# AvalonEnjoyer/pytorch-ViT-paper-replication

Hardware: AMD Instinct MI355X
Metric: images/sec (whole node) ViT-B/16 224px bf16 at 1/2/4/8 MI355X (higher is better)
Workload: dtype bf16; 1 GPU; model=ViT-B/16, global_batch=256, per_gpu_batch=256, seq_len=197, image_size=224, parallelism=dp1, impl=fused, grad_transport=none, optimizer=Adam(wd=0.03 decay group) + clip 1.0 + warmup/linear-decay LR, dropout=0.1 (mlp, embedding)

## Files before the change

### pytorch_vit_paper_replication_amd/csrc/bindings.cpp

```cpp
#include <cstdlib>
#include <algorithm>
#include <map>
#include <torch/extension.h>
#include <c10/hip/HIPStream.h>
#include <hip/hip_runtime.h>

#include "kernels.h"

namespace {

hipStream_t stream() { return c10::hip::getCurrentHIPStream().stream(); }
using ScratchKey = std::pair<int, int64_t>;
ScratchKey scratch_key(int dev) { return std::make_pair(dev, (int64_t)c10::hip::getCurrentHIPStream().id()); }
template <class T>
std::map<ScratchKey, T>& scratch_map() {
  static auto* m = new std::map<ScratchKey, T>();
  return *m;
}
struct SkCounters { torch::Tensor t; };
struct DetWs { torch::Tensor t; };
struct DqWs { torch::Tensor t; };
struct AttnWs { torch::Tensor t; };

int num_cus() {
// ... 931 lines not shown
  TORCH_CHECK(D % H == 0 && pvr_attn_cls_ok((int)N, (int)(D / H)), "attn_cls_fwd: unsupported N / head dim (attn_cls_ok)");
  auto out = torch::empty({B, D}, qkv.options());
  auto lse = torch::empty({B * H}, qkv.options().dtype(torch::kFloat32));
  check(pvr_attn_cls_fwd(bf(qkv, "qkv"), ld_of(qkv, "qkv"), bf_mut(out, "out"), D, f32_mut(lse, "lse"), (int)B, (int)N, (int)H, (int)D,
                         (float)scale, stream()),
        "attn_cls_fwd");
  return {out, lse};
}

std::vector<torch::Tensor> attn_cls_bwd(torch::Tensor dout, torch::Tensor qkv, torch::Tensor out, torch::Tensor lse, int64_t B, int64_t N,
                                        int64_t H, double scale) {
  TORCH_CHECK(qkv.dim() == 2 && qkv.size(0) == B * N && qkv.size(1) % 3 == 0 && H > 0, "attn_cls_bwd: qkv [B*N][3D]");
  const int64_t D = qkv.size(1) / 3;
  TORCH_CHECK(D % H == 0 && pvr_attn_cls_ok((int)N, (int)(D / H)), "attn_cls_bwd: unsupported N / head dim (attn_cls_ok)");
  TORCH_CHECK(dout.dim() == 2 && dout.size(0) == B && dout.size(1) == D && out.dim() == 2 && out.size(0) == B && out.size(1) == D &&
                  lse.numel() == B * H && lse.is_contiguous(),
              "attn_cls_bwd: dout / out [B][D], lse [B*H]");
  auto dqkv = torch::empty({B * N, 3 * D}, qkv.options());
  auto dq0 = torch::empty({B, D}, qkv.options().dtype(torch::kFloat32));
  check(pvr_attn_cls_bwd(bf(qkv, "qkv"), ld_of(qkv, "qkv"), bf(out, "out"), ld_of(out, "out"), bf(dout, "dout"), ld_of(dout, "dout"),
                         f32(lse, "lse"), bf_mut(dqkv, "dqkv"), 3 * D, f32_mut(dq0, "dq0"), (int)B, (int)N, (int)H, (int)D, (float)scale,
                         stream()),
        "attn_cls_bwd");
  return {dqkv, dq0};
}

void attn_cls_dbias(torch::Tensor dq0, torch::Tensor dout, torch::Tensor dbias) {
  TORCH_CHECK(dq0.dim() == 2 && dq0.is_contiguous() && dout.dim() == 2 && dout.size(0) == dq0.size(0) && dout.size(1) == dq0.size(1) &&
                  dbias.is_contiguous() && dbias.numel() == 3 * dq0.size(1),
              "attn_cls_dbias: dq0 f32 [B][D] contiguous, dout bf16 [B][D], dbias f32 [3D]");
  check(pvr_attn_cls_dbias(f32(dq0, "dq0"), bf(dout, "dout"), ld_of(dout, "dout"), f32_mut(dbias, "dbias"), (int)dq0.size(0),
                           (int)dq0.size(1), stream()),
        "attn_cls_dbias");
}

}

extern "C" const char* pvr_src_hash(void);

PYBIND11_MODULE(TORCH_EXTENSION_NAME, m) {
  m.doc() = "MI355X (gfx950) HIP kernels for pytorch_vit_paper_replication_amd";
  m.def("source_hash", []() { return std::string(pvr_src_hash()); },
        "content hash of the csrc/ sources this binary was built from (build.source_hash())");
  m.def("gemm_tail_split", [](int64_t M, int64_t N, int64_t K, int64_t elem_bytes, int64_t max_units) {
    return pvr_gemm_tail_split((int)M, (int)N, (int)K, (int)elem_bytes, (int)max_units); },
    py::arg("M"), py::arg("N"), py::arg("K"), py::arg("elem_bytes"), py::arg("max_units") = 0,
    "K-parts of the split tail round this GEMM shape gets (0: none)");
  m.def("set_attn_dbg", [](torch::Tensor t) { pvr_set_attn_dbg(t.defined() && t.numel() ? t.data_ptr() : nullptr); },
        "diagnostic builds (-DPVR_ATTN_STAMPS): int64 buffer for the attention backward's phase stamps "
        "[workgroup * waves + wave][8] (scripts/attn_stamps.py); a no-op otherwise");
  m.def("set_attn_prep_xcd", &pvr_set_attn_prep_xcd, "attention backward pre-pass: XCD-contiguous (batch, head) pairs (1) or round-robin (0, default); A/B");
  m.def("set_ln_fwd_q8_grid", &pvr_set_ln_fwd_q8_grid, "LayerNorm forward with the e4m3 copy: grid cap in workgroups per CU (A/B)");
  m.def("set_attn_fwd_head_qf", &pvr_set_attn_fwd_head_qf, "whole-head attention forward (dh 64, N <= 256): 16-query fragments per wave (1 = default, 2 = half the LDS reads with 7 waves; A/B)");
  m.def("set_attn_fwd_qg", &pvr_set_attn_fwd_qg, "tiled attention forward: 16-query groups per wave (0 = auto by query padding, 1 = round-3 form, 2 = forced; A/B)");
  m.def("set_fp8_persistent", &pvr_set_fp8_persistent, "fp8 fwd/dgrad GEMMs on the persistent ping-pong: 1 when the epilogue has no per-row input (default), 0 never (A/B)");
  m.def("set_deterministic", &set_deterministic, "deterministic reductions (partial rows + ordered sum) instead of float atomics");
  m.def("deterministic", &deterministic);
  m.def("set_gemm_tail", &set_gemm_tail, "split-K tail of the last dispatch round on (True, default) / off (A/B)");
  m.def("gemm", &gemm,py::arg("A"), py::arg("a_kcontig"), py::arg("B"), py::arg("b_kcontig"), py::arg("C"),
        py::arg("M"), py::arg("N"), py::arg("K"), py::arg("epi"), py::arg("bias"), py::arg("resid"), py::arg("addend"),
        py::arg("addend_period"), py::arg("aux"), py::arg("row_group"), py::arg("row_stride_group"),
        py::arg("row_offset"), py::arg("seed"), py::arg("seed_offset"), py::arg("drop_p"), py::arg("k_split"),
        py::arg("tile_cfg"), py::arg("dbg") = py::none(), py::arg("colsum") = py::none(),
        py::arg("epi_staged") = 0, py::arg("tail_limit") = 0, py::arg("reduce_out") = py::none(), py::arg("reduce_acc") = true,
        py::arg("drop_row_mul") = 0);
  m.def("splitk_timeouts", &splitk_timeouts, py::arg("like"), py::arg("reset") = false);
// ... 40 lines not shown
  m.def("metrics_accum", &metrics_accum);
  m.def("rng_next", &rng_next);
  m.def("zero_f32", &zero_f32);
  m.def("gemm_fp8", &gemm_fp8, py::arg("A"), py::arg("fmt_a"), py::arg("B"), py::arg("fmt_b"), py::arg("C"), py::arg("M"),
        py::arg("N"), py::arg("K"), py::arg("epi"), py::arg("scale_a"), py::arg("scale_b"), py::arg("bias") = py::none(),
        py::arg("resid") = py::none(), py::arg("aux") = py::none(), py::arg("seed") = py::none(), py::arg("seed_offset") = 0,
        py::arg("drop_p") = 0.0, py::arg("colsum") = py::none(), py::arg("q_out") = py::none(), py::arg("q_scale") = py::none(),
        py::arg("q_amax") = py::none(), py::arg("q_fmt") = 0, py::arg("c_skip") = false, py::arg("tail_limit") = 0);
  m.def("fp8_transpose", &fp8_transpose);
  m.def("gemm_fp8_wgrad_mn", &gemm_fp8_wgrad_mn, py::arg("dy8"), py::arg("x8"), py::arg("ws"), py::arg("N"), py::arg("K"),
        py::arg("T"), py::arg("scale_a"), py::arg("scale_b"), py::arg("ksplit"), py::arg("fmt_a") = 1);
  m.def("fp8_quant", &fp8_quant, py::arg("x"), py::arg("y"), py::arg("qscale"), py::arg("amax"), py::arg("fmt"));
  m.def("fp8_dequant", &fp8_dequant, py::arg("x"), py::arg("dscale") = py::none(), py::arg("fmt") = 0);
  m.def("fp8_scale_update", &fp8_scale_update);
  m.def("fp8_quant_t", &fp8_quant_t);
  m.def("gemm_fp8_wgrad", &gemm_fp8_wgrad, py::arg("A8"), py::arg("B8"), py::arg("ws"), py::arg("N"), py::arg("K"), py::arg("Tp"),
        py::arg("scale_a"), py::arg("scale_b"), py::arg("ksplit"), py::arg("fmt_a") = 1);
  m.def("fp8_quant_multi", &fp8_quant_multi, py::arg("segs"), py::arg("nchunks"), py::arg("qscale"), py::arg("amax"), py::arg("fmt"),
        py::arg("amax_only"));
  m.def("attn_fwd", &attn_fwd, py::arg("qkv"), py::arg("B"), py::arg("N"), py::arg("H"), py::arg("scale"),
        py::arg("seed") = py::none(), py::arg("seed_offset") = 0, py::arg("drop_p") = 0.0, py::arg("q_out") = py::none(),
        py::arg("q_scale") = py::none(), py::arg("q_amax") = py::none(), py::arg("q_only") = false);
  m.def("attn_bwd", &attn_bwd, py::arg("dout"), py::arg("qkv"), py::arg("out"), py::arg("lse"), py::arg("B"), py::arg("N"),
        py::arg("H"), py::arg("scale"), py::arg("dbias") = py::none(), py::arg("dbias_part") = py::none(),
        py::arg("seed") = py::none(), py::arg("seed_offset") = 0, py::arg("drop_p") = 0.0, py::arg("q_out") = py::none(),
        py::arg("q_scale") = py::none(), py::arg("q_amax") = py::none(), py::arg("q_only") = false,
        py::arg("q_fmt") = 1);
  m.def("attn_cls_ok", [](int64_t N, int64_t dh) { return pvr_attn_cls_ok((int)N, (int)dh) != 0; },
        "the class-token attention kernels take this token count and head dim");
  m.def("attn_cls_fwd", &attn_cls_fwd, py::arg("qkv"), py::arg("B"), py::arg("N"), py::arg("H"), py::arg("scale"));
  m.def("attn_cls_bwd", &attn_cls_bwd, py::arg("dout"), py::arg("qkv"), py::arg("out"), py::arg("lse"), py::arg("B"), py::arg("N"),
        py::arg("H"), py::arg("scale"));
  m.def("attn_cls_dbias", &attn_cls_dbias);
  m.def("attn_bwd_q8_ok", &attn_bwd_q8_ok, "attn_bwd can write dQKV's e5m2 copy for this shape");
  m.def("arch", []() { return std::string("gfx950"); });
}
```

### pytorch_vit_paper_replication_amd/csrc/kernels.h

```cpp
#pragma once
#include <stdint.h>

#include <hip/hip_runtime_api.h>

#include "gemm_params.h"

namespace pvr {

struct AdamGroup {
  float lr, beta1, beta2, eps, weight_decay;
  float bc1, bc2_sqrt;
  int decoupled;
};
static_assert(sizeof(AdamGroup) == 8 * sizeof(float), "AdamGroup is one float32 [8] row of the group table");

struct DropSite {
  const uint64_t* seed = nullptr; uint64_t offset = 0; uint32_t thr = 0; float scale = 1.f;
};

struct Fp8Copy {
  uint8_t* out = nullptr; int64_t ld = 0; const float* scale = nullptr; unsigned* amax = nullptr; int fmt = 0;
};

struct MixRow {
// ... 107 lines not shown
                               int amax_only, hipStream_t s);
hipError_t pvr_fp8_quant_t(const uint16_t* x, int64_t ldx, uint8_t* y, int64_t ldy, int T, int C, const float* qscale, int fmt,
                           hipStream_t s);
hipError_t pvr_fp8_transpose(const uint8_t* x, int64_t ldx, uint8_t* y, int64_t ldy, int T, int C, hipStream_t s);
hipError_t pvr_fp8_dequant(const uint8_t* x, float* y, int64_t n, const float* dscale, int fmt, hipStream_t s);
hipError_t pvr_fp8_scale_update(float* hist, int H, unsigned* amax, float* qscale, float* dscale, const float* fmax, int s0, int s1,
                                float margin_mul, hipStream_t s);

void pvr_set_attn_fwd_qg(int qg);
void pvr_set_attn_fwd_head_qf(int qf);
void pvr_set_attn_prep_xcd(int on);
void pvr_set_attn_dbg(void* p);
int pvr_attn_head_dim_supported(int dh);
hipError_t pvr_attn_fwd(const uint16_t* qkv, int64_t ld, uint16_t* out, int64_t ld_o, float* lse, int B, int N, int H, int D,
                        float scale, pvr::DropSite drop, pvr::Fp8Copy q8, int q8_only, hipStream_t s);
int pvr_attn_dbias_splits(int B, int NQ);
hipError_t pvr_attn_dbias_reduce(const float* part, float* ws, float* dbias, int B, int H, int NQ, int D, hipStream_t s);
int pvr_attn_bwd_waves(int N);
int pvr_attn_bwd_key_blocks(int N);
int pvr_attn_bwd_needs_dq_acc(int N, int dh, int dbias, int drop, int det);
int64_t pvr_attn_bwd_ws_floats(int B, int N, int H, int D, int dbias, int drop, int det);
int pvr_attn_bwd_q8_ok(int N, int drop);
int pvr_attn_bwd_uses_pipe(int B, int N, int H, int D, int64_t ld, int64_t ld_do, int64_t ld_o, int64_t ld_dq, int drop);
int pvr_attn_bwd_part_rows(int B, int N, int H, int D, int64_t ld, int64_t ld_do, int64_t ld_o, int64_t ld_dq, int drop);
hipError_t pvr_attn_bwd(const pvr::AttnBwdParams* p, hipStream_t s);
int pvr_attn_cls_ok(int N, int dh);
hipError_t pvr_attn_cls_fwd(const uint16_t* qkv, int64_t ld, uint16_t* out, int64_t ld_o, float* lse, int B, int N, int H, int D,
                            float scale, hipStream_t s);
hipError_t pvr_attn_cls_bwd(const uint16_t* qkv, int64_t ld, const uint16_t* o, int64_t ld_o, const uint16_t* dout, int64_t ld_do,
                            const float* lse, uint16_t* dqkv, int64_t ld_dq, float* dq0, int B, int N, int H, int D, float scale,
                            hipStream_t s);
hipError_t pvr_attn_cls_dbias(const float* dq0, const uint16_t* dout, int64_t ld_do, float* dbias, int B, int D, hipStream_t s);

}
```

### pytorch_vit_paper_replication_amd/ops/fused_vit.py

```python
from __future__ import annotations

import math
from typing import List, Optional

import torch
import torch.nn.functional as F

from .. import _ext
from . import gemm

SITE_SHIFT = 32
ATTN_SITE = 1 << 20


DGRAD_TAP = None


def site_drop(seed: Optional[torch.Tensor], site: int, p: float, training: bool):
    if seed is None or not training or p <= 0.0:
        return None
    return (seed, site << SITE_SHIFT, float(p))


def _patch_geometry(C, H, W, patch):
# ... 346 lines not shown
        if q8res is not None:
            pre_q[3] = q8res
        elif fp8_qkv:
            prod = f8d[0].grad_producer(f8d[1], 3)
            if side_db and prod is not None:
                pre_q[3] = gemm.bias_grad(dqkv, gbqkv, quant=prod)
                side_db = False
            else:
                pre_q[3] = f8d[0].grad_quant(dqkv, f8d[1], 3)
        store.on_side(attn_wgrads, dx1, o, dqkv, xn1, do, *(() if db_part is None else (db_part,)), *side8(2, 3))
        dxn1 = dgrad(dqkv, wqkv, 3)
        dx = torch.empty_like(dx2)
        if prev is not None:
            seed, soff, p = gemm._drop_args(prev.drop2)
            dzp = torch.empty_like(dx2) if seed is not None else None
            pf8 = (f8d[0], f8d[1] - 1) if f8d is not None and f8d[1] > 0 else None
            q_kw, q_dz = _ln_grad_quant(pf8, 0, dx.shape, dx.device)
            dz_nostore = (q_dz is not None and dzp is not None and T >= 256 and DGRAD_TAP is None
                          and prev.w2 is not None and store.bf16_t(prev.w2) is not None
                          and pf8[0].wgrad_ready(pf8[1], 0, 3))
            ext.layernorm_bwd(dxn1, D, x, D, mean1, rstd1, ln1w, dx1, D, dx, D, g(ln1w), g(ln1b), T,
                              dsum=g(prev.b2), dz=dzp, seed=seed, seed_offset=soff, drop_p=p, dz_nostore=dz_nostore, **q_kw)
            if dzp is not None:
                _poison(dzp, dz_nostore)
            prev.dz2, prev.dz2_q, prev.done = dzp, q_dz, True
        else:
            ext.layernorm_bwd(dxn1, D, x, D, mean1, rstd1, ln1w, dx1, D, dx, D, g(ln1w), g(ln1b), T)
        store.grad_ready([bo, wo, bqkv, wqkv, ln1w, ln1b])
        return (dx,) + (None,) * (9 + len(params))


CLS_LAST_BLOCK = True


def cls_last_block_ok(N: int, H: int, D: int, f8, dropa) -> bool:
    return (CLS_LAST_BLOCK and f8 is None and gemm._drop_args(dropa)[0] is None
            and D % H == 0 and bool(_ext.ext().attn_cls_ok(N, D // H)))


class EncoderBlockClsFn(torch.autograd.Function):

    @staticmethod
    def forward(ctx, x, B, N, H, eps1, eps2, store, drops, links, *params):
        ext = _ext.ext()
        drop1, drop2, _ = drops
        ln1w, ln1b, wqkv, bqkv, wo, bo, ln2w, ln2b, w1, b1, w2, b2 = params
        T, D = x.shape
        ctx.links = links if links is not None else (None, None)
        M = w1.shape[0]
        scale = 1.0 / math.sqrt(D // H)
        need_bwd = getattr(store, "grad_enabled", True) and any(ctx.needs_input_grad)
        xn1, mean1, rstd1 = ext.layernorm_fwd(x, ln1w, ln1b, eps1, T, D)
        qkv = gemm.linear_fwd(xn1, store.bf16(wqkv), bqkv)
        o, lse = ext.attn_cls_fwd(qkv, B, N, H, scale)
        xc = x.view(B, N, D)[:, 0]
        x1 = gemm.linear_fwd(o, store.bf16(wo), bo, resid=xc)
        xn2, mean2, rstd2 = ext.layernorm_fwd(x1, ln2w, ln2b, eps2, B, D)
        u = torch.empty(B, M, dtype=torch.bfloat16, device=x.device) if need_bwd else None
        h = gemm.linear_fwd(xn2, store.bf16(w1), b1, gelu_aux=u, gelu=True, drop=drop1, drop_row_mul=N)
        x2 = gemm.linear_fwd(h, store.bf16(w2), b2, resid=x1, drop=drop2, drop_row_mul=N)
        if need_bwd:
            ctx.save_for_backward(x, xn1, mean1, rstd1, qkv, o, lse, x1, xn2, mean2, rstd2, u, h)
        ctx.meta = (B, N, H, scale, store, drop2, params)
        return x2

    @staticmethod
    def backward(ctx, dx2):
        ext = _ext.ext()
        det = _ext.deterministic()
        x, xn1, mean1, rstd1, qkv, o, lse, x1, xn2, mean2, rstd2, u, h = ctx.saved_tensors
        B, N, H, scale, store, drop2, params = ctx.meta
        ln1w, ln1b, wqkv, bqkv, wo, bo, ln2w, ln2b, w1, b1, w2, b2 = params
        g = store.grad_dest
        dx2 = dx2.contiguous()
        T, D = x.shape
        _, prev = ctx.links

        def dgrad(dy, w, which, dgelu_aux=None, colsum=None):
            out = gemm.linear_dgrad(dy, store.bf16(w), dgelu_aux=dgelu_aux, wt=store.bf16_t(w), colsum=colsum)
            if DGRAD_TAP is not None:
                DGRAD_TAP(which, out)
            return out

        if drop2 is not None:
            dz2 = torch.empty_like(dx2)
            gemm.bias_grad(dx2, g(b2), drop=drop2, dz=dz2, row_mul=N)
        else:
            dz2 = dx2
            if b2.requires_grad:
                gemm.bias_grad(dx2, g(b2))
        gb1 = g(b1)
        gw2, gw1 = g(w2), g(w1)
        du = dgrad(dz2, w2, 0, dgelu_aux=u, colsum=None if det else gb1)
        if det and gb1 is not None:
            gemm.bias_grad(du, gb1)

        def mlp_wgrads():
            if gw2 is not None:
                gemm.linear_wgrad(dz2, h, gw2)
            if gw1 is not None:
                gemm.linear_wgrad(du, xn2, gw1)

        store.on_side(mlp_wgrads, dz2, h, du, xn2)
        dxn2 = dgrad(du, w1, 1)
        dx1 = torch.empty_like(dx2)
        ext.layernorm_bwd(dxn2, D, x1, D, mean2, rstd2, ln2w, dx2, D, dx1, D, g(ln2w), g(ln2b), B, dsum=g(bo))
        store.grad_ready([w2, b2, w1, b1, ln2w, ln2b])
        gwo, gwqkv, gbqkv = g(wo), g(wqkv), g(bqkv)
        do = dgrad(dx1, wo, 2)
        dqkv, dq0 = ext.attn_cls_bwd(do, qkv, o, lse, B, N, H, scale)

        def attn_wgrads():
            if gbqkv is not None:
                ext.attn_cls_dbias(dq0, do, gbqkv.view(-1))
            if gwo is not None:
                gemm.linear_wgrad(dx1, o, gwo)
            if gwqkv is not None:
                gemm.linear_wgrad(dqkv, xn1, gwqkv)

        store.on_side(attn_wgrads, dx1, o, dqkv, xn1, do, dq0)
        dxn1 = dgrad(dqkv, wqkv, 3)
        dx = torch.empty_like(x)
        if prev is not None:
            seed, soff, p = gemm._drop_args(prev.drop2)
            dzp = torch.empty_like(x) if seed is not None else None
            ext.layernorm_bwd(dxn1, D, x, D, mean1, rstd1, ln1w, dx1, D, dx, D, g(ln1w), g(ln1b), T,
                              dsum=g(prev.b2), dz=dzp, seed=seed, seed_offset=soff, drop_p=p, dres_every=N)
            prev.dz2, prev.dz2_q, prev.done = dzp, None, True
        else:
            ext.layernorm_bwd(dxn1, D, x, D, mean1, rstd1, ln1w, dx1, D, dx, D, g(ln1w), g(ln1b), T, dres_every=N)
        store.grad_ready([bo, wo, bqkv, wqkv, ln1w, ln1b])
        return (dx,) + (None,) * (8 + len(params))


class HeadFn(torch.autograd.Function):

    @staticmethod
    def forward(ctx, tokens, B, N, eps, store, ln_w, ln_b, head_w, head_b):
        ext = _ext.ext()
        logits, xhat, rstd = ext.head_fwd(tokens, B, N, ln_w, ln_b, eps, head_w, head_b)
        ctx.save_for_backward(xhat, rstd)
        ctx.meta = (B, N, store, ln_w, ln_b, head_w, head_b)
        return logits

    @staticmethod
    def backward(ctx, dlogits):
        ext = _ext.ext()
        _ext.deterministic()
        xhat, rstd = ctx.saved_tensors
        B, N, store, ln_w, ln_b, head_w, head_b = ctx.meta
        g = store.grad_dest
        dlogits = dlogits.float().contiguous()
        dtokens = ext.head_bwd(dlogits, xhat, rstd, ln_w, ln_b, head_w, B, N, g(head_w), g(head_b), g(ln_w), g(ln_b))
        store.grad_ready([head_w, head_b, ln_w, ln_b])
# ... 138 lines not shown
```

Before: 7969 images/sec.

## Replace last-block class-token attention with pooled algebraic formulation avoiding full QKV GEMM

In the last transformer block only the class token's output is needed. The full QKV projection over all tokens is replaced with a class-token Q projection, folding Wk into the query (a = scale·q·Wk per head) and Wv into the pooled output. Softmax-weighted pooling over the normalized tokens happens in new HIP kernels, with matching backward kernels for dxn, da and the head-folded weight gradients. This removes the B*N x 3D QKV GEMM and its dgrad/wgrad for that block. In exchange it adds several custom fp32 reduction kernels and uses a different summation order than before.

Measured after the change: 8004 images/sec (median of 6 runs). About the same (+0.4%).

```diff
diff --git a/pytorch_vit_paper_replication_amd/csrc/bindings.cpp b/pytorch_vit_paper_replication_amd/csrc/bindings.cpp
--- a/pytorch_vit_paper_replication_amd/csrc/bindings.cpp
+++ b/pytorch_vit_paper_replication_amd/csrc/bindings.cpp
@@ -987,6 +987,110 @@
   check(pvr_attn_cls_dbias(f32(dq0, "dq0"), bf(dout, "dout"), ld_of(dout, "dout"), f32_mut(dbias, "dbias"), (int)dq0.size(0),
                            (int)dq0.size(1), stream()),
         "attn_cls_dbias");
+}
+
+void cls_pool_check(const char* fn, const torch::Tensor& xn, int64_t B, int64_t N, int64_t H) {
+  TORCH_CHECK(B > 0 && N > 0 && H > 0 && xn.dim() == 2 && xn.size(0) == B * N && xn.is_contiguous(), fn, ": xn [B*N][D] contiguous");
+  TORCH_CHECK(reinterpret_cast<uintptr_t>(xn.data_ptr()) % 8 == 0, fn, ": xn must be 8-byte aligned");
+  TORCH_CHECK(pvr_cls_pool_ok((int)N, (int)xn.size(1), (int)H), fn, ": unsupported N / D / H (cls_pool_ok)");
+}
+void cls_bhd_check(const char* fn, const char* name, const torch::Tensor& t, int64_t B, int64_t H, int64_t D) {
+  TORCH_CHECK(t.dim() == 3 && t.size(0) == B && t.size(1) == H && t.size(2) == D && t.is_contiguous() &&
+                  reinterpret_cast<uintptr_t>(t.data_ptr()) % 16 == 0,
+              fn, ": ", name, " must be f32 [B][H][D] contiguous and 16-byte aligned, got ", t.sizes());
+}
+
+std::vector<torch::Tensor> cls_pool_fwd(torch::Tensor xn, torch::Tensor a, int64_t B, int64_t N, int64_t H, bool want_p) {
+  cls_pool_check("cls_pool_fwd", xn, B, N, H);
+  const int64_t D = xn.size(1);
+  cls_bhd_check("cls_pool_fwd", "a", a, B, H, D);
+  auto f32o = xn.options().dtype(torch::kFloat32);
+  auto pooled = torch::empty({B, H, D}, f32o);
+  auto P = want_p ? torch::empty({B, H, N}, f32o) : torch::empty({0}, f32o);
+  check(pvr_cls_pool_fwd(bf(xn, "xn"), f32(a, "a"), f32_mut(pooled, "pooled"), want_p ? f32_mut(P, "P") : nullptr, (int)B, (int)N,
+                         (int)D, (int)H, stream()),
+        "cls_pool_fwd");
+  return {pooled, P};
+}
+
+std::vector<torch::Tensor> cls_pool_bwd(torch::Tensor xn, torch::Tensor a, torch::Tensor P, torch::Tensor dpooled,
+                                        c10::optional<torch::Tensor> addend, int64_t B, int64_t N, int64_t H, bool want_row0) {
+  cls_pool_check("cls_pool_bwd", xn, B, N, H);
+  const int64_t D = xn.size(1);
+  cls_bhd_check("cls_pool_bwd", "a", a, B, H, D);
+  cls_bhd_check("cls_pool_bwd", "dpooled", dpooled, B, H, D);
+  TORCH_CHECK(P.dim() == 3 && P.size(0) == B && P.size(1) == H && P.size(2) == N && P.is_contiguous(),
+              "cls_pool_bwd: P must be f32 [B][H][N] contiguous, got ", P.sizes());
+  const uint16_t* add = nullptr;
+  int64_t ld_add = 0;
+  if (addend.has_value() && addend->defined()) {
+    TORCH_CHECK(addend->dim() == 2 && addend->size(0) == B && addend->size(1) == D, "cls_pool_bwd: addend must be bf16 [B][D]");
+    add = bf(*addend, "addend");
+    ld_add = ld_of(*addend, "addend");
+  }
+  auto f32o = xn.options().dtype(torch::kFloat32);
+  auto dxn = torch::empty_like(xn);
+  auto da = torch::empty({B, H, D}, f32o);
+  auto row0 = want_row0 ? torch::empty({B, D}, f32o) : torch::empty({0}, f32o);
+  check(pvr_cls_pool_bwd(bf(xn, "xn"), f32(a, "a"), f32(P, "P"), f32(dpooled, "dpooled"), add, ld_add, bf_mut(dxn, "dxn"),
+                         f32_mut(da, "da"), want_row0 ? f32_mut(row0, "row0") : nullptr, (int)B, (int)N, (int)D, (int)H, stream()),
+        "cls_pool_bwd");
+  return {dxn, da, row0};
+}
+
+void cls_pool_row0(torch::Tensor dxn, torch::Tensor row0, torch::Tensor addend, int64_t N) {
+  TORCH_CHECK(row0.dim() == 2 && row0.is_contiguous() && N > 0, "cls_pool_row0: row0 f32 [B][D] contiguous");
+  const int64_t B = row0.size(0), D = row0.size(1);
+  TORCH_CHECK(dxn.dim() == 2 && dxn.is_contiguous() && dxn.size(0) == B * N && dxn.size(1) == D && D % 4 == 0 && addend.dim() == 2 &&
+                  addend.size(0) == B && addend.size(1) == D,
+              "cls_pool_row0: dxn bf16 [B*N][D] contiguous, addend bf16 [B][D], D % 4 == 0");
+  check(pvr_cls_pool_row0(bf_mut(dxn, "dxn"), f32(row0, "row0"), bf(addend, "addend"), ld_of(addend, "addend"), (int)B, (int)N, (int)D,
+                          stream()),
+        "cls_pool_row0");
+}
+
+int64_t cls_head_w(const char* fn, const torch::Tensor& W, int64_t H, int64_t D) {
+  TORCH_CHECK(H > 0 && W.dim() == 2 && W.size(1) == D && W.size(0) % H == 0 && W.size(0) > 0, fn, ": W must be bf16 [H * dh][D]");
+  return W.size(0) / H;
+}
+
+torch::Tensor cls_head_expand(torch::Tensor v, torch::Tensor W, int64_t H, double alpha) {
+  TORCH_CHECK(W.dim() == 2, "cls_head_expand: W must be 2-D");
+  const int64_t D = W.size(1), dh = cls_head_w("cls_head_expand", W, H, D), B = v.dim() == 2 ? v.size(0) : 0;
+  TORCH_CHECK(v.dim() == 2 && B > 0 && v.size(1) == H * dh, "cls_head_expand: v must be bf16 [B][H * dh]");
+  auto out = torch::empty({B, H, D}, v.options().dtype(torch::kFloat32));
+  check(pvr_cls_head_expand(bf(v, "v"), ld_of(v, "v"), bf(W, "W"), ld_of(W, "W"), f32_mut(out, "out"), (int)B, (int)H, (int)D, (int)dh,
+                            (float)alpha, stream()),
+        "cls_head_expand");
+  return out;
+}
+
+std::vector<torch::Tensor> cls_head_contract(torch::Tensor t, torch::Tensor W, c10::optional<torch::Tensor> bias, double alpha,
+                                             bool want_f32) {
+  TORCH_CHECK(t.dim() == 3 && t.is_contiguous() && t.size(0) > 0, "cls_head_contract: t must be f32 [B][H][D] contiguous");
+  const int64_t B = t.size(0), H = t.size(1), D = t.size(2), dh = cls_head_w("cls_head_contract", W, H, D);
+  const float* bp = nullptr;
+  if (bias.has_value() && bias->defined()) {
+    TORCH_CHECK(bias->dim() == 1 && bias->numel() == H * dh && bias->is_contiguous(), "cls_head_contract: bias must be f32 [H * dh]");
+    bp = f32(*bias, "bias");
+  }
+  auto out = torch::empty({B, H * dh}, t.options().dtype(torch::kBFloat16));
+  auto out32 = want_f32 ? torch::empty({B, H * dh}, t.options()) : torch::empty({0}, t.options());
+  check(pvr_cls_head_contract(f32(t, "t"), bf(W, "W"), ld_of(W, "W"), bp, bf_mut(out, "out"), want_f32 ? f32_mut(out32, "out32") : nullptr,
+                              (int)B, (int)H, (int)D, (int)dh, (float)alpha, stream()),
+        "cls_head_contract");
+  return {out, out32};
+}
+
+void cls_head_wgrad(torch::Tensor v, torch::Tensor t, torch::Tensor dW, double alpha) {
+  TORCH_CHECK(t.dim() == 3 && t.is_contiguous() && t.size(0) > 0, "cls_head_wgrad: t must be f32 [B][H][D] contiguous");
+  const int64_t B = t.size(0), H = t.size(1), D = t.size(2);
+  TORCH_CHECK(dW.dim() == 2 && dW.size(1) == D && dW.stride(1) == 1 && dW.size(0) % H == 0 && dW.size(0) > 0 && v.dim() == 2 &&
+                  v.size(0) == B && v.size(1) == dW.size(0),
+              "cls_head_wgrad: dW f32 [H * dh][D] with unit column stride, v bf16 [B][H * dh]");
+  check(pvr_cls_head_wgrad(bf(v, "v"), ld_of(v, "v"), f32(t, "t"), f32_mut(dW, "dW"), dW.stride(0), (int)B, (int)H, (int)D,
+                           (int)(dW.size(0) / H), (float)alpha, stream()),
+        "cls_head_wgrad");
 }
 
 }
@@ -1093,6 +1197,16 @@
   m.def("attn_cls_bwd", &attn_cls_bwd, py::arg("dout"), py::arg("qkv"), py::arg("out"), py::arg("lse"), py::arg("B"), py::arg("N"),
         py::arg("H"), py::arg("scale"));
   m.def("attn_cls_dbias", &attn_cls_dbias);
+  m.def("cls_pool_ok", [](int64_t N, int64_t D, int64_t H) { return pvr_cls_pool_ok((int)N, (int)D, (int)H) != 0; },
+        "True if the pooled class-token attention kernels (csrc/cls_pool.hip) take N tokens, width D, H heads");
+  m.def("cls_pool_fwd", &cls_pool_fwd, py::arg("xn"), py::arg("a"), py::arg("B"), py::arg("N"), py::arg("H"), py::arg("want_p") = true);
+  m.def("cls_pool_bwd", &cls_pool_bwd, py::arg("xn"), py::arg("a"), py::arg("P"), py::arg("dpooled"), py::arg("addend"), py::arg("B"),
+        py::arg("N"), py::arg("H"), py::arg("want_row0") = false);
+  m.def("cls_pool_row0", &cls_pool_row0, py::arg("dxn"), py::arg("row0"), py::arg("addend"), py::arg("N"));
+  m.def("cls_head_expand", &cls_head_expand, py::arg("v"), py::arg("W"), py::arg("H"), py::arg("alpha"));
+  m.def("cls_head_contract", &cls_head_contract, py::arg("t"), py::arg("W"), py::arg("bias"), py::arg("alpha"),
+        py::arg("want_f32") = false);
+  m.def("cls_head_wgrad", &cls_head_wgrad, py::arg("v"), py::arg("t"), py::arg("dW"), py::arg("alpha"));
   m.def("attn_bwd_q8_ok", &attn_bwd_q8_ok, "attn_bwd can write dQKV's e5m2 copy for this shape");
   m.def("arch", []() { return std::string("gfx950"); });
 }
diff --git a/pytorch_vit_paper_replication_amd/csrc/cls_pool.hip b/pytorch_vit_paper_replication_amd/csrc/cls_pool.hip
--- /dev/null
+++ b/pytorch_vit_paper_replication_amd/csrc/cls_pool.hip
@@ -0,0 +1,417 @@
+#include "common.h"
+#include "kernels.h"
+
+namespace pvr {
+namespace {
+
+constexpr int CP_NT = 512;
+constexpr int CP_NTF = 1024;
+constexpr int CP_R = 4;
+constexpr float CP_LOG2E = 1.44269504088896340736f;
+
+PVR_DEV void cp_unpack4(uint2 q, float (&f)[4]) {
+  f[0] = __uint_as_float(q.x << 16);
+  f[1] = __uint_as_float(q.x & 0xFFFF0000u);
+  f[2] = __uint_as_float(q.y << 16);
+  f[3] = __uint_as_float(q.y & 0xFFFF0000u);
+}
+
+template <int HB, int NT>
+PVR_DEV void cp_scores(const uint16_t* __restrict__ X, int N, int D, int H, const float* vec, float* sc, int HP) {
+  const int lane = threadIdx.x & 63, wave = threadIdx.x >> 6;
+  const int nc4 = D >> 2;
+  for (int t0 = wave * CP_R; t0 < N; t0 += (NT / 64) * CP_R) {
+    float acc[CP_R][HB];
+#pragma unroll
+    for (int r = 0; r < CP_R; ++r)
+#pragma unroll
+      for (int j = 0; j < HB; ++j) acc[r][j] = 0.f;
+    for (int c = lane; c < nc4; c += 64) {
+      float xf[CP_R][4];
+#pragma unroll
+      for (int r = 0; r < CP_R; ++r)
+        cp_unpack4(*(const uint2*)(X + (int64_t)min(t0 + r, N - 1) * D + 4 * c), xf[r]);
+#pragma unroll
+      for (int j = 0; j < HB; ++j) {
+        if (j < H) {
+          const float4 v = *(const float4*)(vec + j * D + 4 * c);
+#pragma unroll
+          for (int r = 0; r < CP_R; ++r)
+            acc[r][j] = fmaf(xf[r][3], v.w, fmaf(xf[r][2], v.z, fmaf(xf[r][1], v.y, fmaf(xf[r][0], v.x, acc[r][j]))));
+        }
+      }
+    }
+#pragma unroll
+    for (int r = 0; r < CP_R; ++r)
+#pragma unroll
+      for (int j = 0; j < HB; ++j) {
+        if (j < H) {
+          const float s = wave_sum(acc[r][j]);
+          if (lane == 0 && t0 + r < N) sc[(t0 + r) * HP + j] = s;
+        }
+      }
+  }
+}
+
+template <int HB>
+PVR_DEV void cp_group_reduce(float (&acc)[HB][4], float* buf, int G, int g, int c, int D, int H) {
+  for (int r = 1; r < G; ++r) {
+    __syncthreads();
+    if (g == r) {
+#pragma unroll
+      for (int j = 0; j < HB; ++j)
+        if (j < H) *(float4*)(buf + j * D + 4 * c) = make_float4(acc[j][0], acc[j][1], acc[j][2], acc[j][3]);
+    }
+    __syncthreads();
+    if (g == 0) {
+#pragma unroll
+      for (int j = 0; j < HB; ++j)
+        if (j < H) {
+          const float4 v = *(const float4*)(buf + j * D + 4 * c);
+          acc[j][0] += v.x; acc[j][1] += v.y; acc[j][2] += v.z; acc[j][3] += v.w;
+        }
+    }
+  }
+}
+
+template <int HB>
+__global__ void __launch_bounds__(CP_NTF) cls_pool_fwd_kernel(const uint16_t* __restrict__ xn, const float* __restrict__ a,
+                                                             float* __restrict__ pooled, float* __restrict__ P, int N, int D, int H) {
+  extern __shared__ float4 cp_smem_f[];
+  float* av = (float*)cp_smem_f;
+  float* sc = av + H * D;
+  const int HP = (H + 3) & ~3;
+  const int b = blockIdx.x, tid = threadIdx.x, lane = tid & 63, wave = tid >> 6;
+  const uint16_t* X = xn + (int64_t)b * N * D;
+  for (int i = tid * 4; i < H * D; i += CP_NTF * 4) *(float4*)(av + i) = *(const float4*)(a + (int64_t)b * H * D + i);
+  for (int i = tid; i < N * (HP - H); i += CP_NTF) sc[(i / (HP - H)) * HP + H + i % (HP - H)] = 0.f;
+  __syncthreads();
+  cp_scores<HB, CP_NTF>(X, N, D, H, av, sc, HP);
+  __syncthreads();
+  for (int h = wave; h < H; h += CP_NTF / 64) {
+    float m = -INFINITY;
+    for (int t = lane; t < N; t += 64) m = fmaxf(m, sc[t * HP + h]);
+    m = wave_max(m);
+    float l = 0.f;
+    for (int t = lane; t < N; t += 64) {
+      const float e = __builtin_amdgcn_exp2f((sc[t * HP + h] - m) * CP_LOG2E);
+      sc[t * HP + h] = e;
+      l += e;
+    }
+    l = wave_sum(l);
+    for (int t = lane; t < N; t += 64) {
+      const float p = sc[t * HP + h] / l;
+      sc[t * HP + h] = p;
+      if (P) P[((int64_t)b * H + h) * N + t] = p;
+    }
+  }
+  __syncthreads();
+  const int nc4 = D >> 2, G = CP_NTF / nc4, g = tid / nc4, c = tid % nc4;
+  float acc[HB][4];
+#pragma unroll
+  for (int j = 0; j < HB; ++j) acc[j][0] = acc[j][1] = acc[j][2] = acc[j][3] = 0.f;
+  if (g < G) {
+#pragma unroll 4
+    for (int t = g; t < N; t += G) {
+      float xf[4];
+      cp_unpack4(*(const uint2*)(X + (int64_t)t * D + 4 * c), xf);
+#pragma unroll
+      for (int j4 = 0; j4 < HB / 4; ++j4) {
+        if (4 * j4 < H) {
+          const float4 p4 = *(const float4*)(sc + t * HP + 4 * j4);
+          const float pj[4] = {p4.x, p4.y, p4.z, p4.w};
+#pragma unroll
+          for (int jj = 0; jj < 4; ++jj)
+#pragma unroll
+            for (int k = 0; k < 4; ++k) acc[4 * j4 + jj][k] = fmaf(pj[jj], xf[k], acc[4 * j4 + jj][k]);
+        }
+      }
+    }
+  }
+  cp_group_reduce<HB>(acc, av, G, g, c, D, H);
+  if (g == 0) {
+#pragma unroll
+    for (int j = 0; j < HB; ++j)
+      if (j < H) *(float4*)(pooled + ((int64_t)b * H + j) * D + 4 * c) = make_float4(acc[j][0], acc[j][1], acc[j][2], acc[j][3]);
+  }
+}
+
+template <int HB>
+__global__ void __launch_bounds__(CP_NT) cls_pool_bwd_kernel(const uint16_t* __restrict__ xn, const float* __restrict__ a,
+                                                             const float* __restrict__ P, const float* __restrict__ dpooled,
+                                                             const uint16_t* __restrict__ addend, int64_t ld_add,
+                                                             uint16_t* __restrict__ dxn, float* __restrict__ da,
+                                                             float* __restrict__ row0, int N, int D, int H) {
+  extern __shared__ float4 cp_smem_b[];
+  float* dv = (float*)cp_smem_b;
+  const int HP = (H + 3) & ~3;
+  float* pl = dv + H * D;
+  float* ds = pl + N * HP;
+  const int b = blockIdx.x, tid = threadIdx.x, lane = tid & 63, wave = tid >> 6;
+  const uint16_t* X = xn + (int64_t)b * N * D;
+  for (int i = tid * 4; i < H * D; i += CP_NT * 4) *(float4*)(dv + i) = *(const float4*)(dpooled + (int64_t)b * H * D + i);
+  for (int i = tid; i < H * N; i += CP_NT) pl[(i % N) * HP + i / N] = P[(int64_t)b * H * N + i];
+  for (int i = tid; i < N * (HP - H); i += CP_NT) {
+    const int o = (i / (HP - H)) * HP + H + i % (HP - H);
+    pl[o] = 0.f;
+    ds[o] = 0.f;
+  }
+  __syncthreads();
+  cp_scores<HB, CP_NT>(X, N, D, H, dv, ds, HP);
+  __syncthreads();
+  for (int h = wave; h < H; h += CP_NT / 64) {
+    float d = 0.f;
+    for (int t = lane; t < N; t += 64) d = fmaf(pl[t * HP + h], ds[t * HP + h], d);
+    d = wave_sum(d);
+    for (int t = lane; t < N; t += 64) ds[t * HP + h] = pl[t * HP + h] * (ds[t * HP + h] - d);
+  }
+  __syncthreads();
+  const int nc4 = D >> 2, G = CP_NT / nc4, g = tid / nc4, c = tid % nc4;
+  float acc[HB][4], af[HB][4], df[HB][4];
+#pragma unroll
+  for (int j = 0; j < HB; ++j) {
+    float4 va = make_float4(0.f, 0.f, 0.f, 0.f), vd = va;
+    if (j < H && g < G) {
+      va = *(const float4*)(a + ((int64_t)b * H + j) * D + 4 * c);
+      vd = *(const float4*)(dpooled + ((int64_t)b * H + j) * D + 4 * c);
+    }
+    af[j][0] = va.x; af[j][1] = va.y; af[j][2] = va.z; af[j][3] = va.w;
+    df[j][0] = vd.x; df[j][1] = vd.y; df[j][2] = vd.z; df[j][3] = vd.w;
+    acc[j][0] = acc[j][1] = acc[j][2] = acc[j][3] = 0.f;
+  }
+  if (g < G) {
+#pragma unroll 2
+    for (int t = g; t < N; t += G) {
+      float xf[4], o[4] = {0.f, 0.f, 0.f, 0.f};
+      cp_unpack4(*(const uint2*)(X + (int64_t)t * D + 4 * c), xf);
+#pragma unroll
+      for (int j4 = 0; j4 < HB / 4; ++j4) {
+        if (4 * j4 < H) {
+          const float4 p4 = *(const float4*)(pl + t * HP + 4 * j4);
+          const float4 s4 = *(const float4*)(ds + t * HP + 4 * j4);
+          const float pj[4] = {p4.x, p4.y, p4.z, p4.w}, sj[4] = {s4.x, s4.y, s4.z, s4.w};
+#pragma unroll
+          for (int jj = 0; jj < 4; ++jj)
+#pragma unroll
+            for (int k = 0; k < 4; ++k) {
+              o[k] = fmaf(sj[jj], af[4 * j4 + jj][k], fmaf(pj[jj], df[4 * j4 + jj][k], o[k]));
+              acc[4 * j4 + jj][k] = fmaf(sj[jj], xf[k], acc[4 * j4 + jj][k]);
+            }
+        }
+      }
+      if (t == 0) {
+        if (addend) {
+          float ad[4];
+          cp_unpack4(*(const uint2*)(addend + (int64_t)b * ld_add + 4 * c), ad);
+#pragma unroll
+          for (int k = 0; k < 4; ++k) o[k] += ad[k];
+        }
+        if (row0) *(float4*)(row0 + (int64_t)b * D + 4 * c) = make_float4(o[0], o[1], o[2], o[3]);
+      }
+      *(uint2*)(dxn + ((int64_t)b * N + t) * D + 4 * c) = make_uint2(pack2bf(o[0], o[1]), pack2bf(o[2], o[3]));
+    }
+  }
+  cp_group_reduce<HB>(acc, dv, G, g, c, D, H);
+  if (g == 0) {
+#pragma unroll
+    for (int j = 0; j < HB; ++j)
+      if (j < H) *(float4*)(da + ((int64_t)b * H + j) * D + 4 * c) = make_float4(acc[j][0], acc[j][1], acc[j][2], acc[j][3]);
+  }
+}
+
+__global__ void __launch_bounds__(256) cls_pool_row0_kernel(uint16_t* __restrict__ dxn, const float* __restrict__ row0,
+                                                            const uint16_t* __restrict__ addend, int64_t ld_add, int B, int N, int D) {
+  const int nc4 = D >> 2;
+  const int i = blockIdx.x * 256 + threadIdx.x;
+  if (i >= B * nc4) return;
+  const int b = i / nc4, c = i % nc4;
+  const float4 r = *(const float4*)(row0 + (int64_t)b * D + 4 * c);
+  float ad[4];
+  cp_unpack4(*(const uint2*)(addend + (int64_t)b * ld_add + 4 * c), ad);
+  *(uint2*)(dxn + (int64_t)b * N * D + 4 * c) = make_uint2(pack2bf(r.x + ad[0], r.y + ad[1]), pack2bf(r.z + ad[2], r.w + ad[3]));
+}
+
+constexpr int CH_BT = 4;
+constexpr int CH_NT = 128;
+constexpr int CH_JS = 2;
+constexpr int CH_DH = 128;
+constexpr int CW_JT = 8;
+constexpr int CW_BC = 256;
+
+__global__ void __launch_bounds__(CH_NT) cls_head_expand_kernel(const uint16_t* __restrict__ v, int64_t ld_v, const uint16_t* __restrict__ W,
+                                                                int64_t ld_w, float* __restrict__ out, int B, int H, int D, int dh,
+                                                                float alpha) {
+  __shared__ float vs[CH_DH][CH_BT];
+  const int b0 = blockIdx.x * CH_BT, h = blockIdx.y, tid = threadIdx.x;
+  for (int i = tid; i < CH_BT * dh; i += CH_NT) {
+    const int bi = i / dh, j = i % dh;
+    vs[j][bi] = b0 + bi < B ? bf2f(v[(int64_t)(b0 + bi) * ld_v + h * dh + j]) : 0.f;
+  }
+  __syncthreads();
+  const int cp = blockIdx.z * CH_NT + tid;
+  if (cp >= (D >> 1)) return;
+  float acc[CH_BT][2];
+#pragma unroll
+  for (int i = 0; i < CH_BT; ++i) acc[i][0] = acc[i][1] = 0.f;
+  const uint16_t* wcol = W + (int64_t)h * dh * ld_w + 2 * cp;
+#pragma unroll 8
+  for (int j = 0; j < dh; ++j) {
+    const uint32_t w2 = *(const uint32_t*)(wcol + (int64_t)j * ld_w);
+    const float w0 = __uint_as_float(w2 << 16), w1 = __uint_as_float(w2 & 0xFFFF0000u);
+    const float4 va = *(const float4*)&vs[j][0];
+    const float vv[CH_BT] = {va.x, va.y, va.z, va.w};
+#pragma unroll
+    for (int i = 0; i < CH_BT; ++i) {
+      acc[i][0] = fmaf(vv[i], w0, acc[i][0]);
+      acc[i][1] = fmaf(vv[i], w1, acc[i][1]);
+    }
+  }
+#pragma unroll
+  for (int i = 0; i < CH_BT; ++i)
+    if (b0 + i < B) *(float2*)(out + ((int64_t)(b0 + i) * H + h) * D + 2 * cp) = make_float2(alpha * acc[i][0], alpha * acc[i][1]);
+}
+
+__global__ void __launch_bounds__(256) cls_head_contract_kernel(const float* __restrict__ t, const uint16_t* __restrict__ W, int64_t ld_w,
+                                                                const float* __restrict__ bias, uint16_t* __restrict__ out,
+                                                                float* __restrict__ out32, int B, int H, int D, int dh, float alpha) {
+  extern __shared__ float4 ch_smem[];
+  float* ts = (float*)ch_smem;
+  const int b0 = blockIdx.x * CH_BT, h = blockIdx.y, tid = threadIdx.x, lane = tid & 63, wave = tid >> 6;
+  for (int i = tid * 4; i < CH_BT * D; i += 256 * 4) {
+    const int bi = i / D, d = i % D;
+    *(float4*)(ts + i) = b0 + bi < B ? *(const float4*)(t + ((int64_t)(b0 + bi) * H + h) * D + d) : make_float4(0.f, 0.f, 0.f, 0.f);
+  }
+  __syncthreads();
+  const int HD = H * dh;
+  for (int j = blockIdx.z * 4 + wave; j < dh; j += 4 * CH_JS) {
+    float acc[CH_BT];
+#pragma unroll
+    for (int i = 0; i < CH_BT; ++i) acc[i] = 0.f;
+    const uint16_t* wrow = W + (int64_t)(h * dh + j) * ld_w;
+    for (int c = lane; c < (D >> 2); c += 64) {
+      float wf[4];
+      cp_unpack4(*(const uint2*)(wrow + 4 * c), wf);
+#pragma unroll
+      for (int i = 0; i < CH_BT; ++i) {
+        const float4 tv = *(const float4*)(ts + i * D + 4 * c);
+        acc[i] = fmaf(tv.w, wf[3], fmaf(tv.z, wf[2], fmaf(tv.y, wf[1], fmaf(tv.x, wf[0], acc[i]))));
+      }
+    }
+    const float bj = bias ? bias[h * dh + j] : 0.f;
+#pragma unroll
+    for (int i = 0; i < CH_BT; ++i) {
+      const float s = fmaf(alpha, wave_sum(acc[i]), bj);
+      if (lane == 0 && b0 + i < B) {
+        out[(int64_t)(b0 + i) * HD + h * dh + j] = f2bf(s);
+        if (out32) out32[(int64_t)(b0 + i) * HD + h * dh + j] = s;
+      }
+    }
+  }
+}
+
+__global__ void __launch_bounds__(256) cls_head_wgrad_kernel(const uint16_t* __restrict__ v, int64_t ld_v, const float* __restrict__ t,
+                                                             float* __restrict__ dW, int64_t ld_dw, int B, int H, int D, int dh,
+                                                             float alpha) {
+  __shared__ float vs[CW_BC][CW_JT];
+  const int d = blockIdx.x * 256 + threadIdx.x, j0 = blockIdx.y * CW_JT, h = blockIdx.z, tid = threadIdx.x;
+  float acc[CW_JT];
+#pragma unroll
+  for (int jj = 0; jj < CW_JT; ++jj) acc[jj] = 0.f;
+  for (int bb = 0; bb < B; bb += CW_BC) {
+    __syncthreads();
+    for (int i = tid; i < CW_BC * CW_JT; i += 256) {
+      const int bi = i / CW_JT, jj = i % CW_JT;
+      vs[bi][jj] = bb + bi < B ? bf2f(v[(int64_t)(bb + bi) * ld_v + h * dh + j0 + jj]) : 0.f;
+    }
+    __syncthreads();
+    const int nb = min(CW_BC, B - bb);
+    if (d < D) {
+#pragma unroll 4
+      for (int bi = 0; bi < nb; ++bi) {
+        const float tv = t[((int64_t)(bb + bi) * H + h) * D + d];
+        const float4 va = *(const float4*)&vs[bi][0], vb = *(const float4*)&vs[bi][4];
+        const float vv[CW_JT] = {va.x, va.y, va.z, va.w, vb.x, vb.y, vb.z, vb.w};
+#pragma unroll
+        for (int jj = 0; jj < CW_JT; ++jj) acc[jj] = fmaf(vv[jj], tv, acc[jj]);
+      }
+    }
+  }
+  if (d < D) {
+#pragma unroll
+    for (int jj = 0; jj < CW_JT; ++jj) dW[(int64_t)(h * dh + j0 + jj) * ld_dw + d] += alpha * acc[jj];
+  }
+}
+
+size_t cp_fwd_lds(int N, int D, int H) { return ((size_t)H * D + (size_t)N * ((H + 3) & ~3)) * sizeof(float); }
+size_t cp_bwd_lds(int N, int D, int H) { return ((size_t)H * D + 2 * (size_t)N * ((H + 3) & ~3)) * sizeof(float); }
+
+bool ch_args_ok(int B, int H, int D, int dh) { return B > 0 && H > 0 && D > 0 && D % 4 == 0 && D <= 2048 && dh > 0 && dh <= CH_DH; }
+
+}
+}
+
+extern "C" int pvr_cls_pool_ok(int N, int D, int H) {
+  if (N < 1 || H < 1 || H > 12 || D < 4 || D % H != 0 || D % 4 != 0 || D / 4 > pvr::CP_NT) return 0;
+  const int dh = D / H;
+  if (dh % pvr::CW_JT != 0 || dh > pvr::CH_DH) return 0;
+  return pvr::cp_bwd_lds(N, D, H) <= 65536 ? 1 : 0;
+}
+
+extern "C" hipError_t pvr_cls_pool_fwd(const uint16_t* xn, const float* a, float* pooled, float* P, int B, int N, int D, int H,
+                                       hipStream_t s) {
+  using namespace pvr;
+  if (B <= 0 || !pvr_cls_pool_ok(N, D, H)) return hipErrorInvalidValue;
+  const size_t smem = cp_fwd_lds(N, D, H);
+  if (H <= 4)
+    hipLaunchKernelGGL(cls_pool_fwd_kernel<4>, dim3(B), dim3(CP_NTF), smem, s, xn, a, pooled, P, N, D, H);
+  else
+    hipLaunchKernelGGL(cls_pool_fwd_kernel<12>, dim3(B), dim3(CP_NTF), smem, s, xn, a, pooled, P, N, D, H);
+  return hipGetLastError();
+}
+
+extern "C" hipError_t pvr_cls_pool_bwd(const uint16_t* xn, const float* a, const float* P, const float* dpooled, const uint16_t* addend,
+                                       int64_t ld_add, uint16_t* dxn, float* da, float* row0, int B, int N, int D, int H, hipStream_t s) {
+  using namespace pvr;
+  if (B <= 0 || !pvr_cls_pool_ok(N, D, H) || (addend && (ld_add < D || ld_add % 4 != 0))) return hipErrorInvalidValue;
+  const size_t smem = cp_bwd_lds(N, D, H);
+  if (H <= 4)
+    hipLaunchKernelGGL(cls_pool_bwd_kernel<4>, dim3(B), dim3(CP_NT), smem, s, xn, a, P, dpooled, addend, ld_add, dxn, da, row0, N, D, H);
+  else
+    hipLaunchKernelGGL(cls_pool_bwd_kernel<12>, dim3(B), dim3(CP_NT), smem, s, xn, a, P, dpooled, addend, ld_add, dxn, da, row0, N, D, H);
+  return hipGetLastError();
+}
+
+extern "C" hipError_t pvr_cls_pool_row0(uint16_t* dxn, const float* row0, const uint16_t* addend, int64_t ld_add, int B, int N, int D,
+                                        hipStream_t s) {
+  if (B <= 0 || N <= 0 || D <= 0 || D % 4 != 0 || ld_add < D || ld_add % 4 != 0 || (int64_t)B * (D / 4) > INT32_MAX)
+    return hipErrorInvalidValue;
+  hipLaunchKernelGGL(pvr::cls_pool_row0_kernel, dim3((B * (D / 4) + 255) / 256), dim3(256), 0, s, dxn, row0, addend, ld_add, B, N, D);
+  return hipGetLastError();
+}
+
+extern "C" hipError_t pvr_cls_head_expand(const uint16_t* v, int64_t ld_v, const uint16_t* W, int64_t ld_w, float* out, int B, int H,
+                                          int D, int dh, float alpha, hipStream_t s) {
+  using namespace pvr;
+  if (!ch_args_ok(B, H, D, dh) || ld_v < (int64_t)H * dh || ld_w < D || ld_w % 2 != 0 || H > 65535) return hipErrorInvalidValue;
+  hipLaunchKernelGGL(cls_head_expand_kernel, dim3((B + CH_BT - 1) / CH_BT, H, ((D >> 1) + CH_NT - 1) / CH_NT), dim3(CH_NT), 0, s, v, ld_v, W,
+                     ld_w, out, B, H, D, dh, alpha);
+  return hipGetLastError();
+}
+
+extern "C" hipError_t pvr_cls_head_contract(const float* t, const uint16_t* W, int64_t ld_w, const float* bias, uint16_t* out,
+                                            float* out32, int B, int H, int D, int dh, float alpha, hipStream_t s) {
+  using namespace pvr;
+  if (!ch_args_ok(B, H, D, dh) || ld_w < D || ld_w % 4 != 0 || H > 65535) return hipErrorInvalidValue;
+  const size_t smem = (size_t)CH_BT * D * sizeof(float);
+  hipLaunchKernelGGL(cls_head_contract_kernel, dim3((B + CH_BT - 1) / CH_BT, H, CH_JS), dim3(256), smem, s, t, W, ld_w, bias, out, out32, B, H, D,
+                     dh, alpha);
+  return hipGetLastError();
+}
+
+extern "C" hipError_t pvr_cls_head_wgrad(const uint16_t* v, int64_t ld_v, const float* t, float* dW, int64_t ld_dw, int B, int H, int D,
+                                         int dh, float alpha, hipStream_t s) {
+  using namespace pvr;
+  if (!ch_args_ok(B, H, D, dh) || dh % CW_JT != 0 || ld_v < (int64_t)H * dh || ld_dw < D || H > 65535) return hipErrorInvalidValue;
+  hipLaunchKernelGGL(cls_head_wgrad_kernel, dim3((D + 255) / 256, dh / CW_JT, H), dim3(256), 0, s, v, ld_v, t, dW, ld_dw, B, H, D, dh, alpha);
+  return hipGetLastError();
+}
diff --git a/pytorch_vit_paper_replication_amd/csrc/kernels.h b/pytorch_vit_paper_replication_amd/csrc/kernels.h
--- a/pytorch_vit_paper_replication_amd/csrc/kernels.h
+++ b/pytorch_vit_paper_replication_amd/csrc/kernels.h
@@ -163,4 +163,17 @@
                             hipStream_t s);
 hipError_t pvr_attn_cls_dbias(const float* dq0, const uint16_t* dout, int64_t ld_do, float* dbias, int B, int D, hipStream_t s);
 
+int pvr_cls_pool_ok(int N, int D, int H);
+hipError_t pvr_cls_pool_fwd(const uint16_t* xn, const float* a, float* pooled, float* P, int B, int N, int D, int H, hipStream_t s);
+hipError_t pvr_cls_pool_bwd(const uint16_t* xn, const float* a, const float* P, const float* dpooled, const uint16_t* addend,
+                            int64_t ld_add, uint16_t* dxn, float* da, float* row0, int B, int N, int D, int H, hipStream_t s);
+hipError_t pvr_cls_pool_row0(uint16_t* dxn, const float* row0, const uint16_t* addend, int64_t ld_add, int B, int N, int D,
+                             hipStream_t s);
+hipError_t pvr_cls_head_expand(const uint16_t* v, int64_t ld_v, const uint16_t* W, int64_t ld_w, float* out, int B, int H, int D,
+                               int dh, float alpha, hipStream_t s);
+hipError_t pvr_cls_head_contract(const float* t, const uint16_t* W, int64_t ld_w, const float* bias, uint16_t* out, float* out32,
+                                 int B, int H, int D, int dh, float alpha, hipStream_t s);
+hipError_t pvr_cls_head_wgrad(const uint16_t* v, int64_t ld_v, const float* t, float* dW, int64_t ld_dw, int B, int H, int D, int dh,
+                              float alpha, hipStream_t s);
+
 }
diff --git a/pytorch_vit_paper_replication_amd/ops/fused_vit.py b/pytorch_vit_paper_replication_amd/ops/fused_vit.py
--- a/pytorch_vit_paper_replication_amd/ops/fused_vit.py
+++ b/pytorch_vit_paper_replication_amd/ops/fused_vit.py
@@ -402,6 +402,12 @@
 
 CLS_LAST_BLOCK = True
 
+CLS_POOLED_ATTN = True
+
+
+def cls_pooled_attn_ok(N: int, D: int, H: int) -> bool:
+    return CLS_POOLED_ATTN and bool(_ext.ext().cls_pool_ok(N, D, H))
+
 
 def cls_last_block_ok(N: int, H: int, D: int, f8, dropa) -> bool:
     return (CLS_LAST_BLOCK and f8 is None and gemm._drop_args(dropa)[0] is None
@@ -421,8 +427,19 @@
         scale = 1.0 / math.sqrt(D // H)
         need_bwd = getattr(store, "grad_enabled", True) and any(ctx.needs_input_grad)
         xn1, mean1, rstd1 = ext.layernorm_fwd(x, ln1w, ln1b, eps1, T, D)
-        qkv = gemm.linear_fwd(xn1, store.bf16(wqkv), bqkv)
-        o, lse = ext.attn_cls_fwd(qkv, B, N, H, scale)
+        pooled_attn = cls_pooled_attn_ok(N, D, H)
+        if pooled_attn:
+            w16 = store.bf16(wqkv)
+            xnc = xn1.view(B, N, D)[:, 0].contiguous()
+            q = gemm.linear_fwd(xnc, w16[:D], bqkv[:D])
+            a = ext.cls_head_expand(q, w16[D:2 * D], H, scale)
+            pooled, P = ext.cls_pool_fwd(xn1, a, B, N, H, want_p=need_bwd)
+            o = ext.cls_head_contract(pooled, w16[2 * D:], bqkv[2 * D:], 1.0)[0]
+            attn_saved = (xnc, q, a, P, pooled)
+        else:
+            qkv = gemm.linear_fwd(xn1, store.bf16(wqkv), bqkv)
+            o, lse = ext.attn_cls_fwd(qkv, B, N, H, scale)
+            attn_saved = (qkv, lse)
         xc = x.view(B, N, D)[:, 0]
         x1 = gemm.linear_fwd(o, store.bf16(wo), bo, resid=xc)
         xn2, mean2, rstd2 = ext.layernorm_fwd(x1, ln2w, ln2b, eps2, B, D)
@@ -430,15 +447,16 @@
         h = gemm.linear_fwd(xn2, store.bf16(w1), b1, gelu_aux=u, gelu=True, drop=drop1, drop_row_mul=N)
         x2 = gemm.linear_fwd(h, store.bf16(w2), b2, resid=x1, drop=drop2, drop_row_mul=N)
         if need_bwd:
-            ctx.save_for_backward(x, xn1, mean1, rstd1, qkv, o, lse, x1, xn2, mean2, rstd2, u, h)
+            ctx.save_for_backward(x, xn1, mean1, rstd1, o, x1, xn2, mean2, rstd2, u, h, *attn_saved)
         ctx.meta = (B, N, H, scale, store, drop2, params)
+        ctx.pooled_attn = pooled_attn
         return x2
 
     @staticmethod
     def backward(ctx, dx2):
         ext = _ext.ext()
         det = _ext.deterministic()
-        x, xn1, mean1, rstd1, qkv, o, lse, x1, xn2, mean2, rstd2, u, h = ctx.saved_tensors
+        x, xn1, mean1, rstd1, o, x1, xn2, mean2, rstd2, u, h, *attn_saved = ctx.saved_tensors
         B, N, H, scale, store, drop2, params = ctx.meta
         ln1w, ln1b, wqkv, bqkv, wo, bo, ln2w, ln2b, w1, b1, w2, b2 = params
         g = store.grad_dest
@@ -478,18 +496,42 @@
         store.grad_ready([w2, b2, w1, b1, ln2w, ln2b])
         gwo, gwqkv, gbqkv = g(wo), g(wqkv), g(bqkv)
         do = dgrad(dx1, wo, 2)
-        dqkv, dq0 = ext.attn_cls_bwd(do, qkv, o, lse, B, N, H, scale)
-
-        def attn_wgrads():
-            if gbqkv is not None:
-                ext.attn_cls_dbias(dq0, do, gbqkv.view(-1))
-            if gwo is not None:
-                gemm.linear_wgrad(dx1, o, gwo)
-            if gwqkv is not None:
-                gemm.linear_wgrad(dqkv, xn1, gwqkv)
-
-        store.on_side(attn_wgrads, dx1, o, dqkv, xn1, do, dq0)
-        dxn1 = dgrad(dqkv, wqkv, 3)
+        if ctx.pooled_attn:
+            xnc, q, a, P, pooled = attn_saved
+            w16 = store.bf16(wqkv)
+            dpooled = ext.cls_head_expand(do, w16[2 * D:], H, 1.0)
+            dxn1, da, row0 = ext.cls_pool_bwd(xn1, a, P, dpooled, None, B, N, H, want_row0=True)
+            dq, dq32 = ext.cls_head_contract(da, w16[D:2 * D], None, scale, want_f32=True)
+
+            def attn_wgrads():
+                if gbqkv is not None:
+                    ext.attn_cls_dbias(dq32, do, gbqkv.view(-1))
+                if gwo is not None:
+                    gemm.linear_wgrad(dx1, o, gwo)
+                if gwqkv is not None:
+                    gemm.linear_wgrad(dq, xnc, gwqkv[:D])
+                    ext.cls_head_wgrad(q, da, gwqkv[D:2 * D], scale)
+                    ext.cls_head_wgrad(do, pooled, gwqkv[2 * D:], 1.0)
+
+            store.on_side(attn_wgrads, dx1, o, xnc, q, da, pooled, do, dq, dq32)
+            wt = store.bf16_t(wqkv)
+            ext.cls_pool_row0(dxn1, row0, gemm.linear_dgrad(dq, w16[:D], wt=None if wt is None else wt[:, :D]), N)
+            if DGRAD_TAP is not None:
+                DGRAD_TAP(3, dxn1)
+        else:
+            qkv, lse = attn_saved
+            dqkv, dq0 = ext.attn_cls_bwd(do, qkv, o, lse, B, N, H, scale)
+
+            def attn_wgrads():
+                if gbqkv is not None:
+                    ext.attn_cls_dbias(dq0, do, gbqkv.view(-1))
+                if gwo is not None:
+                    gemm.linear_wgrad(dx1, o, gwo)
+                if gwqkv is not None:
+                    gemm.linear_wgrad(dqkv, xn1, gwqkv)
+
+            store.on_side(attn_wgrads, dx1, o, dqkv, xn1, do, dq0)
+            dxn1 = dgrad(dqkv, wqkv, 3)
         dx = torch.empty_like(x)
         if prev is not None:
             seed, soff, p = gemm._drop_args(prev.drop2)
```
